# martasumyk/hyperspectral_super-resolution

Measured on AMD Instinct MI355X. Metric: Mpixel*bands/s fused (SRF + deg-3 per-band LSQ fit + apply), higher is better.
Workload: dtype f32

## Files before the change

hyperspectral_super-resolution_amd/csrc/hsr_exec.hip:

```cpp
#include <new>
#include <vector>

#include "hsr_common.h"
#include "hsr_solve.h"
#include "hsr_sync_dev.h"

struct hsr_step_plan {
  hsr_step_desc d;
  int32_t k0[HSR_MAX_BANDS], klen[HSR_MAX_BANDS];
  int32_t slots;
};

enum { kTwoSlot = 0, kFused = 1, kExchange = 2, kGroup = 3 };

struct pipe_slot {
  hsr_step_plan* p = nullptr;
  hipEvent_t ev_k1 = nullptr;
  hipEvent_t ev_fit = nullptr;
  bool pending = false;
  bool fitted = false;
  bool exchanged = false;
  unsigned int seq = 0;
};

struct hsr_pipeline {
  std::vector<pipe_slot> slot;
  int kind = kTwoSlot;
  int nslots = 0;
  int group_T = 0;
  double* group_moments = nullptr;
  double* group_total = nullptr;
  double* group_coeffs = nullptr;
  hipStream_t side = nullptr;
  int64_t n = 0;
  int exchange = 0;
  unsigned int* sync = nullptr;
  unsigned int tickets = 0;
  hsr_exchange x{};
  unsigned int published = 0;
  int deferred = -1;
  int deferred_solve = 0;
  double* host_moments[4] = {};
  struct host_job { hsr_pipeline* pl; double* values; int32_t count; } host_jobs[4] = {};
  volatile int host_error = 0;
};

namespace {

__global__ __launch_bounds__(64) void gate_kernel(const unsigned int* word, unsigned int target, unsigned int* err, unsigned int code) {
  if (threadIdx.x == 0) hsr::wait_word_at_least(word, target, err, code);
}

__global__ __launch_bounds__(64) void publish_add_kernel(unsigned int* word, unsigned int n) {
  if (threadIdx.x == 0) __hip_atomic_fetch_add(word, n, __ATOMIC_RELAXED, __HIP_MEMORY_SCOPE_AGENT);
}

__global__ __launch_bounds__(256) void rehearsal_collective_kernel(int us, unsigned int* sink) {
  __shared__ unsigned int lds[12288];
  lds[threadIdx.x] = threadIdx.x;
  __syncthreads();
  const unsigned long long t0 = hsr::sync_realtime();
  while (hsr::sync_realtime() - t0 < (unsigned long long)us * 100ull) __builtin_amdgcn_s_sleep(8);
  if (lds[(threadIdx.x * 7) & 255] == 0xffffffffu) *sink = 1u;
}

__global__ __launch_bounds__(64) void solve_publish_kernel(const double* __restrict__ moments, int nb, int deg, long long min_count,
                                                           double* coeffs, int do_solve, unsigned int* ready, unsigned int value,
                                                           const unsigned int* gate_word, unsigned int gate_target, unsigned int* err) {
  const int b = threadIdx.x;
  if (do_solve && b < nb) {
    double c[HSR_MAX_DEG + 1];
    hsr::solve_band(moments + (size_t)b * hsr::moment_count(deg), deg, min_count, c);
    for (int j = 0; j <= deg; ++j)
      __hip_atomic_store(coeffs + (size_t)b * (deg + 1) + j, c[j], __ATOMIC_RELAXED, __HIP_MEMORY_SCOPE_AGENT);
  }
  asm volatile("s_waitcnt vmcnt(0)" ::: "memory");
  __syncthreads();
// ... 61 lines not shown

extern "C" int hsr_step_run(hsr_step_plan* p, const void* cube_dev, const float* real_dev, const uint8_t* mask_dev,
                            hsr_stream_t stream) {
  HSR_REQUIRE(p && cube_dev && real_dev, HSR_ERR_INVALID, "hsr_step_run: NULL argument");
  hipStream_t s = (hipStream_t)stream;
  int rc = run_k1(p, cube_dev, real_dev, mask_dev, s);
  if (rc != HSR_OK) return rc;
  rc = hsr_moments_reduce_solve(p->d.partials_dev, p->slots, p->d.nb, p->d.deg, p->d.min_count, p->d.moments_dev, p->d.coeffs_dev, s);
  if (rc != HSR_OK) return rc;
  return run_apply(p, p->d.coeffs_dev, mask_dev, s);
}

extern "C" int hsr_step_run_k1(hsr_step_plan* p, const void* cube_dev, const float* real_dev, const uint8_t* mask_dev,
                               hsr_stream_t stream) {
  HSR_REQUIRE(p && cube_dev && real_dev, HSR_ERR_INVALID, "hsr_step_run_k1: NULL argument");
  return run_k1(p, cube_dev, real_dev, mask_dev, (hipStream_t)stream);
}

extern "C" int hsr_step_run_reduce(hsr_step_plan* p, hsr_stream_t stream) {
  HSR_REQUIRE(p, HSR_ERR_INVALID, "hsr_step_run_reduce: NULL plan");
  return hsr_moments_reduce(p->d.partials_dev, p->slots, p->d.nb, p->d.deg, p->d.moments_dev, stream);
}

extern "C" int hsr_step_run_solve(hsr_step_plan* p, hsr_stream_t stream) {
  HSR_REQUIRE(p, HSR_ERR_INVALID, "hsr_step_run_solve: NULL plan");
  return hsr_poly_solve(p->d.moments_dev, p->d.nb, p->d.deg, p->d.min_count, p->d.coeffs_dev, stream);
}

extern "C" int hsr_step_run_apply(hsr_step_plan* p, const uint8_t* mask_dev, hsr_stream_t stream) {
  HSR_REQUIRE(p, HSR_ERR_INVALID, "hsr_step_run_apply: NULL plan");
  return run_apply(p, p->d.coeffs_dev, mask_dev, (hipStream_t)stream);
}

static int pipeline_new(hsr_step_plan* const* sl, int nslots, int kind, hsr_stream_t side_stream, hsr_pipeline** out, const char* who) {
  HSR_REQUIRE(out, HSR_ERR_INVALID, "%s: NULL argument", who);
  for (int i = 0; i < nslots; ++i) {
    HSR_REQUIRE(sl[i], HSR_ERR_INVALID, "%s: NULL plan", who);
    for (int k = 0; k < i; ++k) {
      HSR_REQUIRE(sl[i] != sl[k], HSR_ERR_INVALID, "%s: distinct plans needed", who);
      const hsr_step_desc &a = sl[i]->d, &b = sl[k]->d;
      HSR_REQUIRE(kind == kTwoSlot || (a.partials_dev != b.partials_dev && a.moments_dev != b.moments_dev && a.coeffs_dev != b.coeffs_dev &&
                                       a.pseudo_dev != b.pseudo_dev && a.matched_dev != b.matched_dev),
                  HSR_ERR_INVALID, "%s: plans %d and %d share a work buffer (partials / moments / coefficients / images must be distinct)", who, k, i);
    }
  }
  HSR_REQUIRE(side_stream != nullptr, HSR_ERR_INVALID, "%s: the side stream must be a real stream, not the default one", who);
  hsr_pipeline* pl = new (std::nothrow) hsr_pipeline();
  HSR_REQUIRE(pl, HSR_ERR_INVALID, "%s: out of host memory", who);
  pl->slot.resize(nslots);
  for (int k = 0; k < nslots; ++k) pl->slot[k].p = sl[k];
  pl->kind = kind;
  pl->nslots = nslots;
  pl->side = (hipStream_t)side_stream;
  bool ok = true;
  if (kind != kTwoSlot)
    ok = hipMalloc(&pl->sync, 8 * sizeof(unsigned int)) == hipSuccess && hipMemset(pl->sync, 0, 8 * sizeof(unsigned int)) == hipSuccess &&
         hipDeviceSynchronize() == hipSuccess;
  if (kind == kTwoSlot || kind == kExchange)
    for (pipe_slot& s : pl->slot)
      ok = ok && hipEventCreateWithFlags(&s.ev_fit, hipEventDisableTiming) == hipSuccess &&
           (kind != kTwoSlot || hipEventCreateWithFlags(&s.ev_k1, hipEventDisableTiming) == hipSuccess);
  if (!ok) {
    (void)hipGetLastError();
    hsr_pipeline_destroy(pl);
    hsr::set_error("%s: could not create the pipeline's device words or events", who);
    return HSR_ERR_HIP;
  }
  *out = pl;
  return HSR_OK;
}

extern "C" int hsr_pipeline_create(hsr_step_plan* slot0, hsr_step_plan* slot1, hsr_stream_t side_stream, int32_t exchange,
                                   hsr_pipeline** out) {
  hsr_step_plan* sl[2] = {slot0, slot1};
  int rc = pipeline_new(sl, 2, kTwoSlot, side_stream, out, "hsr_pipeline_create");
  if (rc == HSR_OK) (*out)->exchange = exchange ? 1 : 0;
  return rc;
}
// ... 44 lines not shown
    for (int k = 0; k < 4; ++k) {
      if (hipHostMalloc(&pl->host_moments[k], bytes, hipHostMallocDefault) != hipSuccess) {
        (void)hipGetLastError();
        hsr_pipeline_destroy(pl);
        hsr::set_error("%s: could not allocate the pinned staging of the host transport", who);
        return HSR_ERR_HIP;
      }
      pl->host_jobs[k] = {pl, pl->host_moments[k], (int32_t)(bytes / sizeof(double))};
    }
  }
  *out = pl;
  return HSR_OK;
}

extern "C" int hsr_pipeline_create_group(hsr_step_plan* const* slots, int32_t nslots, int32_t group_tiles, double* group_moments_dev,
                                         double* group_total_dev, double* group_coeffs_dev, hsr_stream_t side_stream, hsr_pipeline** out) {
  const char* who = "hsr_pipeline_create_group";
  HSR_REQUIRE(slots && out && group_moments_dev && group_total_dev && group_coeffs_dev, HSR_ERR_INVALID, "%s: NULL argument", who);
  HSR_REQUIRE(group_tiles >= 2 && group_tiles <= 64 && nslots == group_tiles + 2, HSR_ERR_INVALID,
              "%s: groups of 2 .. 64 tiles and group_tiles + 2 plans needed (got %d tiles, %d plans)", who, group_tiles, nslots);
  int rc = fused_geometry(slots, nslots, who);
  if (rc != HSR_OK) return rc;
  hsr_pipeline* pl = nullptr;
  rc = pipeline_new(slots, nslots, kGroup, side_stream, &pl, who);
  if (rc != HSR_OK) return rc;
  pl->group_T = group_tiles;
  pl->group_moments = group_moments_dev;
  pl->group_total = group_total_dev;
  pl->group_coeffs = group_coeffs_dev;
  *out = pl;
  return HSR_OK;
}

extern "C" void hsr_pipeline_destroy(hsr_pipeline* pl) {
  if (!pl) return;
  if (pl->kind == kExchange) (void)hipStreamSynchronize(pl->side);
  for (pipe_slot& s : pl->slot) {
    if (s.ev_k1) (void)hipEventDestroy(s.ev_k1);
    if (s.ev_fit) (void)hipEventDestroy(s.ev_fit);
  }
  for (int k = 0; k < 4; ++k)
    if (pl->host_moments[k]) (void)hipHostFree(pl->host_moments[k]);
  if (pl->sync) (void)hipFree(pl->sync);
  delete pl;
}

static inline pipe_slot& slot_of(hsr_pipeline* pl, int64_t tile) { return pl->slot[tile % pl->nslots]; }

static void host_sum_trampoline(void* arg) {
  auto* j = static_cast<hsr_pipeline::host_job*>(arg);
  if (j->pl->x.host_sum(j->pl->x.host_user, j->values, j->count) != 0) j->pl->host_error = 1;
}

static int launch_solve_publish(hsr_pipeline* pl, bool with_gate) {
  const pipe_slot& s = pl->slot[pl->deferred];
  const hsr_step_desc& d = s.p->d;
  hipLaunchKernelGGL(solve_publish_kernel, dim3(1), dim3(64), 0, pl->side, d.moments_dev, d.nb, d.deg, (long long)d.min_count, d.coeffs_dev,
                     pl->deferred_solve, pl->sync + 4 + pl->deferred, s.seq, with_gate ? pl->sync + 1 : nullptr, pl->published, pl->sync + 2);
  HSR_LAUNCH_CHECK("solve_publish_kernel");
  pl->deferred = -1;
  return HSR_OK;
}

static int enqueue_exchange(hsr_pipeline* pl, int k) {
  const hsr_step_desc& d = pl->slot[k].p->d;
  const int64_t nmom = (int64_t)d.nb * hsr::moment_count(d.deg);
  int rc = HSR_OK;
  if (pl->deferred >= 0) {
// ... 180 lines not shown
  rc = run_apply(s.p, s.p->d.coeffs_dev, mask, main);
  s.pending = false;
  return rc;
}

static int submit_two_slot(hsr_pipeline* pl, const void* cube_dev, const float* real_dev, const uint8_t* mask_dev,
                           const uint8_t* prev_mask_dev, hipStream_t main, int32_t* finished_slot, void* k1_begin_event,
                           void* k1_end_event) {
  const int cur = (int)(pl->n % 2);
  pipe_slot &s = pl->slot[cur], &prev = pl->slot[cur ^ 1];
  int rc = HSR_OK;
  if (k1_begin_event) rc = hsr::check_hip(hipEventRecord((hipEvent_t)k1_begin_event, main), "hsr_pipeline: record K1 begin");
  if (rc == HSR_OK) rc = run_k1(s.p, cube_dev, real_dev, mask_dev, main);
  if (rc == HSR_OK && k1_end_event) rc = hsr::check_hip(hipEventRecord((hipEvent_t)k1_end_event, main), "hsr_pipeline: record K1 end");
  if (rc != HSR_OK) return rc;
  if (prev.pending) {
    rc = finish_two_slot(prev, prev_mask_dev, main);
    if (rc != HSR_OK) return rc;
    if (finished_slot) *finished_slot = cur ^ 1;
  }
  rc = hsr::check_hip(hipEventRecord(s.ev_k1, main), "hsr_pipeline: record K1");
  if (rc == HSR_OK) rc = hsr::check_hip(hipStreamWaitEvent(pl->side, s.ev_k1, 0), "hsr_pipeline: side stream wait");
  if (rc == HSR_OK && !pl->exchange) {
    const hsr_step_desc& d = s.p->d;
    rc = hsr_moments_reduce_solve(d.partials_dev, s.p->slots, d.nb, d.deg, d.min_count, d.moments_dev, d.coeffs_dev, pl->side);
    if (rc == HSR_OK) rc = hsr::check_hip(hipEventRecord(s.ev_fit, pl->side), "hsr_pipeline: record fit");
  }
  if (rc != HSR_OK) return rc;
  s.pending = true;
  pl->n += 1;
  return HSR_OK;
}

extern "C" int hsr_pipeline_submit(hsr_pipeline* pl, const void* cube_dev, const float* real_dev, const uint8_t* mask_dev,
                                   const uint8_t* prev_mask_dev, hsr_stream_t main_stream, int32_t* finished_slot,
                                   void* k1_begin_event, void* k1_end_event) {
  HSR_REQUIRE(pl && cube_dev && real_dev, HSR_ERR_INVALID, "hsr_pipeline_submit: NULL argument");
  const int cur = (int)(pl->n % pl->nslots);
  HSR_REQUIRE(!pl->slot[cur].pending, HSR_ERR_INVALID, "hsr_pipeline_submit: slot %d still holds an unfinished tile", cur);
  if (finished_slot) *finished_slot = -1;
  hipStream_t main = (hipStream_t)main_stream;
  if (pl->kind == kTwoSlot) return submit_two_slot(pl, cube_dev, real_dev, mask_dev, prev_mask_dev, main, finished_slot, k1_begin_event, k1_end_event);
  return submit_fused(pl, cube_dev, real_dev, mask_dev, prev_mask_dev, main, finished_slot, k1_begin_event, k1_end_event);
}

extern "C" int hsr_pipeline_fit_done(hsr_pipeline* pl) {
  HSR_REQUIRE(pl && pl->n > 0 && pl->kind == kTwoSlot, HSR_ERR_INVALID, "hsr_pipeline_fit_done: nothing submitted, or not a two-slot pipeline");
  return hsr::check_hip(hipEventRecord(slot_of(pl, pl->n - 1).ev_fit, pl->side), "hsr_pipeline: record fit");
}

extern "C" int hsr_pipeline_flush(hsr_pipeline* pl, const uint8_t* mask_dev, hsr_stream_t main_stream, int32_t* finished_slot) {
  HSR_REQUIRE(pl, HSR_ERR_INVALID, "hsr_pipeline_flush: NULL pipeline");
  if (finished_slot) *finished_slot = -1;
  const int S = pl->nslots;
  for (int64_t i = pl->n >= S - 1 ? pl->n - (S - 1) : 0; i < pl->n; ++i) {
    pipe_slot& s = slot_of(pl, i);
    if (!s.pending) continue;
    const int rc = pl->kind == kTwoSlot ? finish_two_slot(s, mask_dev, (hipStream_t)main_stream)
                                        : finish_fused(pl, i, mask_dev, (hipStream_t)main_stream);
    if (rc == HSR_OK && finished_slot) *finished_slot = (int)(i % S);
    return rc;
  }
  return HSR_OK;
}

extern "C" int64_t hsr_pipeline_count(const hsr_pipeline* pl) { return pl ? pl->n : -1; }

extern "C" int hsr_pipeline_status(hsr_pipeline* pl, hsr_stream_t main_stream, uint32_t* sync_error_out) {
  HSR_REQUIRE(pl && sync_error_out, HSR_ERR_INVALID, "hsr_pipeline_status: NULL argument");
  *sync_error_out = 0;
  int rc = hsr::check_hip(hipStreamSynchronize((hipStream_t)main_stream), "hsr_pipeline_status: caller's stream");
  if (rc == HSR_OK) rc = hsr::check_hip(hipStreamSynchronize(pl->side), "hsr_pipeline_status: side stream");
  if (rc != HSR_OK || !pl->sync) return rc;
  unsigned int code = 0;
  rc = hsr::check_hip(hipMemcpy(&code, pl->sync + 2, sizeof code, hipMemcpyDeviceToHost), "hsr_pipeline_status: read the error word");
  *sync_error_out = code | (pl->host_error ? 16u : 0u);
  return rc;
}
```

hyperspectral_super-resolution_amd/s2_emit/_native.py:

```python
from __future__ import annotations

import ctypes as C
import os
from typing import Optional

_HERE = os.path.dirname(os.path.abspath(__file__))
_DEFAULT_SO = os.path.join(os.path.dirname(_HERE), "lib", "libhsr_mi355x.so")

HSR_OK = 0
HSR_MAX_BANDS = 16
HSR_MAX_DEG = 4
HSR_MAX_APPLY_DEG = 8
HSR_MAX_SPECTRAL = 560
HSR_TILE_PIXELS = 64
HSR_SRF_U16_FAST = 1
HSR_MAX_PARTIALS = 4096
HSR_FIT_GROUPS = 64
HSR_FIT_TICKETS = 65
PLANAR = "planar"
PIXMAJOR = "pixmajor"


class HsrUnavailable(RuntimeError):
    """The HIP extension (or a GPU to run it on) is not available."""
# ... 120 lines not shown
                                _i32, _vp, _vp, _vp, _i32, _vp]),
    "hsr_pair_stats": (C.c_int, [_vp, _vp, _i64, _i32, _vp, _vp, _vp, _vp, _i32, _vp]),
    "hsr_pair_expand_f64": (C.c_int, [_vp, _i64, _vp, _vp, _i64, _vp, _i64, _vp, _i64, _i64, _i32, _i32, _i32, _f64, _vp, _i64,
                                      _i64, _i32, _i32, _vp]),
    "hsr_gram_f64_batched": (C.c_int, [_vp, _i64, _i32, _i32, _i64, _i64, _vp, _i64, _vp, _i64, _i64, _i32, _vp]),
    "hsr_ridge_assemble_batched": (C.c_int, [_vp, _i64, _i64, _i32, _i32, _i32, _f64, _vp, _i32, _i64, _vp, _i64, _i64, _vp, _i32,
                                             _vp]),
    "hsr_chol_solve_f64_batched": (C.c_int, [_vp, _i64, _i32, _i64, _vp, _i64, _i32, _i64, _vp, _vp, _i32, _vp]),
    "hsr_ridge_finish_batched": (C.c_int, [_vp, _i64, _i32, _i32, _i32, _vp, _i64, _i64, _vp, _vp, _i64, _i32, _i32, _vp, _vp,
                                           _i64, _vp, _i64, _vp, _vp, _i64, _vp, _vp, _i32, _vp]),
    "hsr_polyfeat_predict_cube_batched": (C.c_int, [_vp, _i64, _i64, _i64, _vp, _vp, _i64, _i64, _i32, _i32, _vp, _i64, _i64, _vp,
                                                    _i64, _i32, _i32, _i32, _f32, _i32, _vp, _i64, _i64, _i32, _vp]),
    "hsr_pair_report_work_bytes": (C.c_size_t, [_i64, _i32]),
    "hsr_pair_report_f64": (C.c_int, [_vp, _i64, _i64, _i32, _i64, _vp, _i64, _vp, _i64, _i64, _i32, _vp, _i64, _vp, _i64, _i32, _vp,
                                      _vp, _i64, _vp, _vp, _i64, _i32, _vp]),
    "hsr_block_mean": (C.c_int, [_vp, _i32, _i64, _i64, _i32, _i32, _i32, _i32, _f32, _vp, _i64, _i64, _vp]),
    "hsr_bilinear_upsample": (C.c_int, [_vp, _i64, _i64, _i32, _i32, _i32, _i32, _vp, _i64, _i64, _vp]),
    "hsr_bilinear_upsample_mask_hist": (C.c_int, [_vp, _i64, _i64, _i32, _i32, _i32, _i32, _vp, _vp, _vp, _vp]),
    "hsr_probe_read": (C.c_int, [_vp, _i64, _i32, _vp, _vp]),
    "hsr_srf_last_launch": (C.c_int, [_pi32, _pi32, C.POINTER(_i64)]),
    "hsr_srf_kernel_instance": (C.c_int, [_i32, _i32]),
    "hsr_poly_last_launch": (C.c_int, [C.c_char_p, _i32]),
    "hsr_polyfeat_predict_kernel": (C.c_int, [_i32, _i32, _i32, _i32]),
    "hsr_step_plan_create": (C.c_int, [C.POINTER(StepDesc), C.POINTER(_vp)]),
    "hsr_step_plan_destroy": (None, [_vp]),
    "hsr_step_plan_slots": (C.c_int, [_vp]),
    "hsr_step_run": (C.c_int, [_vp, _vp, _vp, _vp, _vp]),
    "hsr_step_run_k1": (C.c_int, [_vp, _vp, _vp, _vp, _vp]),
    "hsr_step_run_reduce": (C.c_int, [_vp, _vp]),
    "hsr_step_run_solve": (C.c_int, [_vp, _vp]),
    "hsr_step_run_apply": (C.c_int, [_vp, _vp, _vp]),
    "hsr_pipeline_create": (C.c_int, [_vp, _vp, _vp, _i32, C.POINTER(_vp)]),
    "hsr_pipeline_create_fused": (C.c_int, [_vp, _vp, _vp, _vp, _i32, C.POINTER(_vp)]),
    "hsr_pipeline_destroy": (None, [_vp]),
    "hsr_pipeline_submit": (C.c_int, [_vp, _vp, _vp, _vp, _vp, _vp, _pi32, _vp, _vp]),
    "hsr_pipeline_fit_done": (C.c_int, [_vp]),
    "hsr_pipeline_flush": (C.c_int, [_vp, _vp, _vp, _pi32]),
    "hsr_pipeline_count": (_i64, [_vp]),
    "hsr_pipeline_create_exchange": (C.c_int, [C.POINTER(_vp), _vp, C.POINTER(Exchange), C.POINTER(_vp)]),
    "hsr_pipeline_status": (C.c_int, [_vp, _vp, C.POINTER(C.c_uint32)]),
    "hsr_pipeline_create_group": (C.c_int, [C.POINTER(_vp), _i32, _i32, _vp, _vp, _vp, _vp, C.POINTER(_vp)]),
    "hsr_srf_fused_launch_supported": (C.c_int, [_i32, _i32, _i32, _pi32, _pi32, _i64, _i32, _popt]),
    "hsr_comm_available": (C.c_int, []),
    "hsr_comm_version": (C.c_int, []),
    "hsr_comm_unique_id": (C.c_int, [_vp]),
    "hsr_comm_init": (C.c_int, [_i32, _i32, _vp, C.POINTER(_vp)]),
    "hsr_comm_destroy": (C.c_int, [_vp]),
    "hsr_comm_rank": (C.c_int, [_vp]),
    "hsr_comm_ranks": (C.c_int, [_vp]),
    "hsr_allreduce_f64": (C.c_int, [_vp, _vp, _i64, _vp]),
    "hsr_reduce_f64": (C.c_int, [_vp, _vp, _i64, _i32, _vp]),
    "hsr_allreduce_u32": (C.c_int, [_vp, _vp, _i64, _vp]),
    "hsr_bcast": (C.c_int, [_vp, _vp, _i64, _i32, _vp]),
}

_lib: Optional[C.CDLL] = None
_lib_path: Optional[str] = None


def library_path() -> str:
    return os.environ.get("HSR_LIBRARY", _DEFAULT_SO)


def load() -> C.CDLL:
    global _lib, _lib_path
    if _lib is not None:
# ... 33 lines not shown
```

hyperspectral_super-resolution_amd/s2_emit/fusion.py:

```python
from __future__ import annotations

from dataclasses import dataclass
from typing import Dict, List, Optional, Tuple

import numpy as np

from . import _engine as eng
from . import _native as nat

COEFF_SYNC_MODES = ("local", "allreduce", "broadcast")
_HOST_GROUPS: Dict[int, object] = {}


def _tkey(t):
    return (t.data_ptr(), tuple(t.shape), tuple(t.stride()), str(t.dtype), str(t.device))


@dataclass
class FusionOutput:
    names: List[str]
    pseudo: object
    moments: object
    coeffs: object
    matched: object
    layout: str = nat.PIXMAJOR

    def band(self, which, image="matched"):
        i = self.names.index(which) if isinstance(which, str) else int(which)
        img = getattr(self, image)
        return img[i] if self.layout == nat.PLANAR else img[:, i]

    def planes(self, image="matched"):
        img = getattr(self, image)
        nb = len(self.names)
        return img if self.layout == nat.PLANAR else img[:, :nb].t().contiguous()


class BatchOutput:

    def __init__(self, names, tb):
        self.names, self._tb = list(names), tb
        self.pseudo, self.matched = tb.pseudo, tb.matched
        self.moments, self.coeffs = tb.moments, tb.coeffs
# ... 4 lines not shown

    def tile(self, i: int) -> FusionOutput:
        tb = self._tb
        return FusionOutput(self.names, tb.tile_rows(i, "pseudo"), tb.moments[i], tb.coeffs[i], tb.tile_rows(i, "matched"),
                            nat.PIXMAJOR)


def exchange_moments(moments, coeffs_solver, group=None, mode: str = "allreduce"):
    import torch.distributed as dist
    if mode not in COEFF_SYNC_MODES:
        raise ValueError(f"mode must be one of {COEFF_SYNC_MODES}, got {mode!r}")
    world = dist.get_world_size(group) if (dist.is_available() and dist.is_initialized()) else 0
    if mode == "local" or world == 0:
        return moments, coeffs_solver(moments)
    if mode == "allreduce":
        dist.all_reduce(moments, op=dist.ReduceOp.SUM, group=group)
        return moments, coeffs_solver(moments)
    root = dist.get_global_rank(group, 0) if group is not None else 0
    dist.reduce(moments, dst=root, op=dist.ReduceOp.SUM, group=group)
    coeffs = coeffs_solver(moments)
    dist.broadcast(coeffs, src=root, group=group)
    return moments, coeffs


class SpectralFusion:

    def __init__(self, emit_w, srf_dict, good_mask=None, deg: int = 3, min_valid: Optional[float] = 0.0,
                 min_count: int = 50, clip: bool = True, apply_mask: bool = False, device=None,
                 group=None, coeff_sync: str = "allreduce", layout: str = nat.PIXMAJOR,
                 force_exchange: bool = False, tile_scale=None, tile_nodata: Optional[int] = eng.TILE_NODATA,
                 reserved_cus: Optional[int] = None, tile_pixels: int = 0, u16_single_buffer: bool = False,
                 u16_fast: bool = False, placement_trials: int = 0, fused_fit: bool = False,
                 placement_pitch_gb: float = eng.PLACEMENT_PITCH_GB, placement_budget_gb: Optional[float] = None,
                 side_stream=None, fuse_apply: bool = False, comm=None, rehearsal_collective=None, group_tiles: int = 1):
        torch = nat.require_gpu()
        self.tile_scale, self.tile_nodata = tile_scale, tile_nodata
        if not 1 <= deg <= nat.HSR_MAX_DEG:
            raise ValueError(f"deg must be in [1, {nat.HSR_MAX_DEG}], got {deg}")
        if coeff_sync not in COEFF_SYNC_MODES:
            raise ValueError(f"coeff_sync must be one of {COEFF_SYNC_MODES}")
        self.device = torch.device(device if device is not None else f"cuda:{torch.cuda.current_device()}")
        self.table = eng.build_srf_table(emit_w, srf_dict, good_mask)
        if self.table.nb == 0:
            raise ValueError("no band of srf_dict has support on the (masked) EMIT wavelength grid")
        if self.table.nb > nat.HSR_MAX_BANDS:
            raise ValueError(f"at most {nat.HSR_MAX_BANDS} supported bands per fusion plan")
        self.deg, self.min_count, self.clip, self.apply_mask = deg, int(min_count), bool(clip), bool(apply_mask)
        self.min_valid = float("-inf") if min_valid is None else float(min_valid)
        self.group, self.coeff_sync = group, coeff_sync
        if layout not in (nat.PIXMAJOR, nat.PLANAR):
            raise ValueError(f"layout must be {nat.PIXMAJOR!r} or {nat.PLANAR!r}")
        self.layout = layout
        self.force_exchange = bool(force_exchange)
        if reserved_cus is None:
            reserved_cus = 8 if self._exchanges() else 0
        self.opts = eng.srf_options(tile_pixels, reserved_cus, u16_single_buffer, u16_fast)
        self.u16_single_buffer = bool(u16_single_buffer)
        self._batches: Dict[tuple, object] = {}
        self.placement_trials = max(0, int(placement_trials))
        self.placement_pitch_gb = float(placement_pitch_gb)
        self.placement_budget_gb = None if placement_budget_gb is None else float(placement_budget_gb)
        self.placement_log: Dict[int, list] = {}
        self._placement_stats: Dict[str, float] = {}
        self.fused_fit = bool(fused_fit)
        self._pipe = None
        self.fused_fallback = None
        self.side_stream = side_stream
        self.side_stream_log = None
        self.fuse_apply = bool(fuse_apply)
        self.group_tiles = int(group_tiles)
        if not 1 <= self.group_tiles <= 64:
            raise ValueError("group_tiles must be in [1, 64]")
        self._comm = comm
        self.rehearsal_collective = rehearsal_collective
        self._host_cb = None
        self._backlog: List[FusionOutput] = []
        self._native: Dict[tuple, object] = {}
        self._native_handles: list = []
        self._pipe_images: Dict[int, list] = {}
        self._pipe_matched: Dict[int, list] = {}
        self.ws = eng.MomentWorkspace(self.device, self.table.nb, deg)
        self.table.device_weights(self.device)
        self._buf: Dict[int, Tuple[object, object]] = {}

    @property
    def names(self) -> List[str]:
        return list(self.table.supported)

    def _buffers(self, npix: int, probe=None):
        torch = nat.require_gpu()
        if npix not in self._buf:
            nb = self.table.nb
            pseudo = eng.alloc_image(torch, nb, npix, self.layout, self.device)
            if probe is not None and self.placement_trials > 1 and npix >= (1 << 16):
                pseudo = self._place(npix, pseudo, probe)
            self._buf[npix] = (pseudo, eng.alloc_image(torch, nb, npix, self.layout, self.device))
        return self._buf[npix]

    @property
    def placement_held_gb(self) -> float:
        return float(self._placement_stats.get("held_gb", 0.0))

    def _trials(self, first, make, probe, cap=None, candidate_bytes: int = 0):
        n = self.placement_trials if cap is None else min(cap, self.placement_trials)
        return eng.placement_search(first, make, probe, n, self.placement_pitch_gb, self.device, self.placement_budget_gb,
                                    candidate_bytes, self._placement_stats)

    def _place(self, npix: int, first, probe, count: int = 1):
        torch = nat.require_gpu()
        nb = self.table.nb
        one = lambda: eng.alloc_image(torch, nb, npix, self.layout, self.device)
        if count == 1:
            keep, times = self._trials(first, one, probe, cap=4, candidate_bytes=first.numel() * 4)
        else:
            keep, times = self._trials(list(first), lambda: [one() for _ in range(count)], lambda c: probe(c[0]), cap=4,
                                       candidate_bytes=count * first[0].numel() * 4)
        self.placement_log[npix] = times
        return keep

    def place_inputs(self, cube, real, mask=None):
        torch = nat.require_gpu()
        npix = cube.numel() // cube.shape[-1]
        if self.placement_trials <= 1 or npix in self._buf:
            return cube, real, {}
        nb = self.table.nb

        def images():
            return [eng.alloc_image(torch, nb, npix, self.layout, self.device) for _ in range(4 if self.fuse_apply else 3)]

        def make():
            return (cube.clone(), real.clone(), images())

        def k1(cand):
            c, r, outs = cand
            rr, rl = self._real_image(r, npix)
            eng.srf_integrate_moments(c, self.table, rr, self.deg, self.ws, mask, self.min_valid, self.min_valid, out=outs[0],
                                      reduce=False, layout=self.layout, real_layout=rl, scale=self.tile_scale,
                                      nodata=self.tile_nodata, opts=self.opts)
        first = (cube, real, images())
        cand_bytes = cube.numel() * cube.element_size() + real.numel() * 4 + 4 * npix * eng.padded_row(nb) * 4
        (cube, real, outs), times = self._trials(first, make, k1, candidate_bytes=cand_bytes)
        self._buf[npix] = (outs[0], eng.alloc_image(torch, nb, npix, self.layout, self.device))
        self._pipe_images[npix] = outs[1:]
        self.placement_log[npix] = times
        return cube, real, {"joint_ms": times}

    def place_mosaic(self, tiles, oversample: float = 12.0, pitch_gb: float = 0.0):
        torch = nat.require_gpu()
        tiles = [(c, r) for c, r in tiles]
        T = len(tiles)
        if self.placement_trials <= 1 or T == 0:
            return tiles, {}
        c0, r0 = tiles[0]
        npix = c0.numel() // c0.shape[-1]
        img = eng.alloc_image(torch, self.table.nb, npix, self.layout, self.device)

        def k1(cand):
            c, r = cand
            rr, rl = self._real_image(r, npix)
            eng.srf_integrate_moments(c, self.table, rr, self.deg, self.ws, None, self.min_valid, self.min_valid, out=img, reduce=False,
                                      layout=self.layout, real_layout=rl, scale=self.tile_scale, nodata=self.tile_nodata, opts=self.opts)
        cand_bytes = c0.numel() * c0.element_size() + r0.numel() * 4
        per = pitch_gb * (1 << 30) + cand_bytes
        free, _ = torch.cuda.mem_get_info(self.device)
        budget = 0.5 * free if self.placement_budget_gb is None else min(self.placement_budget_gb * (1 << 30), free)
        count = int(min(max(T, oversample * T), max(T, budget // per)))
        pitch = pitch_gb
        ranked = eng.placement_rank(lambda: (c0.clone(), r0.clone()), k1, count, pitch, self.device, self.placement_budget_gb, cand_bytes,
                                    self._placement_stats, retime=2 * T)
        ranked += [((c, r), float("inf")) for c, r in tiles[:max(0, T - len(ranked))]]
        order = sorted(range(len(ranked)), key=lambda i: ranked[i][1])[:T]
        kept = []
        for (c, r), i in zip(tiles, order):
# ... 452 lines not shown

    def _pipe_build(self, cube, real, mask, key):
        torch = nat.require_gpu()
        import ctypes as C
        lib = nat.load()
        if self._pipe is not None:
            self._backlog = self.drain()
            old, self._pipe = self._pipe, None
            self._drop_handles(old["handles"])
        npix = cube.numel() // cube.shape[-1]
        real2, real_layout = self._real_image(real, npix)
        if not (real2.is_cuda and real2.dtype == torch.float32):
            raise ValueError("real must be a float32 GPU image with one value per pixel and band")
        eng._as_cube2d(cube)
        nb = self.table.nb

        def probe(img):
            eng.srf_integrate_moments(cube, self.table, real2, self.deg, self.ws, mask, self.min_valid, self.min_valid,
                                      out=img, reduce=False, layout=self.layout, real_layout=real_layout,
                                      scale=self.tile_scale, nodata=self.tile_nodata, opts=self.opts)
        placed = list(self._pipe_images.pop(npix, []))
        if len(placed) < 2:
            placed = [eng.alloc_image(torch, nb, npix, self.layout, self.device) for _ in range(2)]
            if self.placement_trials > 1 and npix >= (1 << 16):
                placed = self._place(npix, placed, probe, count=2)
        exchange = self._exchanges()
        if self.group_tiles > 1 and (exchange or not self.fuse_apply or self.layout != nat.PIXMAJOR):
            raise ValueError("group_tiles > 1 needs fuse_apply=True, the pixel-major layout and no exchange (multi-rank mosaics: fuse_mosaic)")
        if not (self.fuse_apply and self.layout == nat.PIXMAJOR and
                (cube.dtype == torch.float32 or (cube.data_ptr() % 16 == 0 and not self.u16_single_buffer))):
            form = "two"
        else:
            form = "group" if self.group_tiles > 1 else ("exchange" if exchange else "fused")
        nslots = {"two": 2, "fused": 3, "exchange": 4, "group": self.group_tiles + 2}[form]
        while len(placed) < nslots:
            placed.append(eng.alloc_image(torch, nb, npix, self.layout, self.device))
        slots, outs, handles = [], [], []
        placed_m = list(self._pipe_matched.pop(npix, []))
        for k in range(nslots):
            ws = eng.MomentWorkspace(self.device, nb, self.deg)
            matched = placed_m[k] if k < len(placed_m) else eng.alloc_image(torch, nb, npix, self.layout, self.device)
            h, keep = self._native_plan(cube, real2, real_layout, placed[k], matched, ws)
            handles.append(("plan", h))
            slots.append(dict(plan=h, ws=ws, keep=keep, mask=None))
            outs.append(FusionOutput(self.names, placed[k], ws.moments, ws.coeffs, matched, self.layout))
        side = (self.side_stream if self.side_stream is not None else
                torch.cuda.Stream(device=self.device) if form in ("fused", "group") else
                self._pick_side_stream(slots, cube, real2, mask))
        ph = C.c_void_p()
        plans = [sl["plan"] for sl in slots]
        transport = gbuf = None
        if form == "group":
            T, M = self.group_tiles, 3 * self.deg + 2
            gbuf = (torch.zeros((2, T, nb, M), dtype=torch.float64, device=self.device), torch.zeros((2, nb, M), dtype=torch.float64, device=self.device),
                    torch.zeros((2, nb, self.deg + 1), dtype=torch.float64, device=self.device))
            nat.check(lib.hsr_pipeline_create_group((C.c_void_p * nslots)(*plans), nslots, T, gbuf[0].data_ptr(), gbuf[1].data_ptr(),
                                                    gbuf[2].data_ptr(), C.c_void_p(side.cuda_stream), C.byref(ph)), "hsr_pipeline_create_group")
        elif form != "two":
            if form == "exchange":
                x, transport = self._exchange_desc()
                rc = lib.hsr_pipeline_create_exchange((C.c_void_p * 4)(*plans), C.c_void_p(side.cuda_stream), C.byref(x), C.byref(ph))
            else:
                rc = lib.hsr_pipeline_create_fused(*plans, C.c_void_p(side.cuda_stream), 0, C.byref(ph))
            if rc != nat.HSR_OK:
                form, transport = "two", None
                self.fused_fallback = lib.hsr_last_error().decode("utf-8", "replace")
                self._drop_handles(handles[2:])
                slots, outs, handles = slots[:2], outs[:2], handles[:2]
                if self.side_stream is None:
                    side = self._pick_side_stream(slots, cube, real2, mask)
        if form == "two":
            nat.check(lib.hsr_pipeline_create(slots[0]["plan"], slots[1]["plan"], C.c_void_p(side.cuda_stream), 1 if exchange else 0,
                                              C.byref(ph)), "hsr_pipeline_create")
        self._native_handles.append(("pipe", ph))
        handles.append(("pipe", ph))
        self._pipe = dict(key=key, npix=npix, h=ph, slots=slots, outs=outs, side=side, side_handle=C.c_void_p(side.cuda_stream),
                          exchange=exchange, n=0, fin=C.c_int32(-1), fused=form != "two", S=len(slots), inflight=[], handles=handles,
                          c_exchange=form == "exchange", transport=transport, group=gbuf, done=0)
        return self._pipe

    @staticmethod
    def _event_handle(ev, stream):
        if not ev.cuda_event:
            ev.record(stream)
        import ctypes as C
        return C.c_void_p(ev.cuda_event)

    def submit(self, cube, real, mask=None, k1_events=None) -> Optional[FusionOutput]:
        torch = nat.require_gpu()
        import ctypes as C
        lib = nat._lib or nat.load()
        key = (tuple(cube.shape), cube.dtype, tuple(real.shape), tuple(real.stride()), real.dtype,
               cube.dtype == torch.float32 or cube.data_ptr() % 16 == 0)
        st = self._pipe
        if st is None or st["key"] != key:
            st = self._pipe_build(cube, real, mask, key)
        if not (cube.is_contiguous() and cube.device == self.device and real.device == self.device):
            raise ValueError("cube must be a contiguous tensor on the plan's GPU, real on the same GPU")
        if mask is not None and not (mask.dtype == torch.uint8 and mask.numel() == st["npix"] and mask.is_contiguous()
                                     and mask.device == self.device):
            raise ValueError("mask must be a contiguous uint8 tensor with one byte per pixel")
        S = st["S"]
        cur = st["n"] % S
        prev_mask = st["slots"][st["inflight"][0]]["mask"] if len(st["inflight"]) == S - 1 else None
        fin = st["fin"]
        with eng._launch(cube) as stream:
            e0 = e1 = None
            if k1_events is not None:
                ts = torch.cuda.current_stream(self.device)
                e0, e1 = self._event_handle(k1_events[0], ts), self._event_handle(k1_events[1], ts)
            nat.check(lib.hsr_pipeline_submit(st["h"], cube.data_ptr(), real.data_ptr(), None if mask is None else mask.data_ptr(),
                                              None if prev_mask is None else prev_mask.data_ptr(), stream, C.byref(fin), e0, e1),
                      "hsr_pipeline_submit")
            slot = st["slots"][cur]
            slot["mask"] = mask
            slot["ws"].slots = lib.hsr_step_plan_slots(slot["plan"])
            if st["exchange"] and not st["c_exchange"]:
                sh = st["side_handle"]
                with torch.cuda.stream(st["side"]):
                    nat.check(lib.hsr_step_run_reduce(slot["plan"], sh), "hsr_step_run_reduce")

                    def solve(_m, _p=slot["plan"], _ws=slot["ws"]):
                        nat.check(lib.hsr_step_run_solve(_p, sh), "hsr_step_run_solve")
                        return _ws.coeffs
                    exchange_moments(slot["ws"].moments, solve, self.group, self.coeff_sync)
                nat.check(lib.hsr_pipeline_fit_done(st["h"]), "hsr_pipeline_fit_done")
        st["n"] += 1
        st["inflight"].append(cur)
        out = None
        if fin.value >= 0:
            st["inflight"].remove(fin.value)
            st["slots"][fin.value]["mask"] = None
            out = self._finished(st, fin.value)
        if self._backlog:
            if out is not None:
                self._backlog.append(out)
            out = self._backlog.pop(0)
# ... 162 lines not shown
```

include/hsr.h:

```cpp
#ifndef HSR_H_
#define HSR_H_

#include <stddef.h>
#include <stdint.h>

#ifdef __cplusplus
extern "C" {
#endif

#define HSR_ABI_VERSION 5

#define HSR_OK 0
#define HSR_ERR_INVALID 1
#define HSR_ERR_UNSUPPORTED 2
#define HSR_ERR_HIP 3

#define HSR_MAX_BANDS 16
#define HSR_MAX_DEG 4
#define HSR_MAX_APPLY_DEG 8
#define HSR_MAX_SPECTRAL 560
#define HSR_TILE_PIXELS 64
#define HSR_MAX_PARTIALS 4096


// ... 295 lines not shown
  const int32_t* klen;
  int32_t nb, deg;
  float* pseudo_dev;
  int64_t out_bs, out_ps;
  int64_t real_bs, real_ps;
  float min_x, min_y;
  double* partials_dev;
  double* moments_dev;
  double* coeffs_dev;
  int64_t min_count;
  float* matched_dev;
  int64_t matched_bs, matched_ps;
  int32_t apply_mask;
  int32_t clip;
  hsr_srf_options opts;
} hsr_step_desc;
typedef struct hsr_step_plan hsr_step_plan;
typedef struct hsr_pipeline hsr_pipeline;

int hsr_step_plan_create(const hsr_step_desc* desc, hsr_step_plan** plan_out);
void hsr_step_plan_destroy(hsr_step_plan* plan);
int hsr_step_plan_slots(const hsr_step_plan* plan);
int hsr_step_run(hsr_step_plan* plan, const void* cube_dev, const float* real_dev, const uint8_t* mask_dev,
                 hsr_stream_t stream);
int hsr_step_run_k1(hsr_step_plan* plan, const void* cube_dev, const float* real_dev, const uint8_t* mask_dev,
                    hsr_stream_t stream);
int hsr_step_run_reduce(hsr_step_plan* plan, hsr_stream_t stream);
int hsr_step_run_solve(hsr_step_plan* plan, hsr_stream_t stream);
int hsr_step_run_apply(hsr_step_plan* plan, const uint8_t* mask_dev, hsr_stream_t stream);
int hsr_pipeline_create(hsr_step_plan* slot0, hsr_step_plan* slot1, hsr_stream_t side_stream, int32_t exchange,
                        hsr_pipeline** pipeline_out);
int hsr_pipeline_create_fused(hsr_step_plan* slot0, hsr_step_plan* slot1, hsr_step_plan* slot2, hsr_stream_t side_stream,
                              int32_t exchange, hsr_pipeline** pipeline_out);
void hsr_pipeline_destroy(hsr_pipeline* pipeline);
int hsr_pipeline_submit(hsr_pipeline* pipeline, const void* cube_dev, const float* real_dev, const uint8_t* mask_dev,
                        const uint8_t* prev_mask_dev, hsr_stream_t main_stream, int32_t* finished_slot,
                        void* k1_begin_event, void* k1_end_event);
int hsr_pipeline_fit_done(hsr_pipeline* pipeline);
int hsr_pipeline_flush(hsr_pipeline* pipeline, const uint8_t* mask_dev, hsr_stream_t main_stream, int32_t* finished_slot);
int64_t hsr_pipeline_count(const hsr_pipeline* pipeline);

#define HSR_COMM_ID_BYTES 128
typedef struct hsr_comm hsr_comm;
int hsr_comm_available(void);
int hsr_comm_version(void);
int hsr_comm_unique_id(void* id_out);
int hsr_comm_init(int32_t rank, int32_t nranks, const void* unique_id, hsr_comm** comm_out);
int hsr_comm_destroy(hsr_comm* comm);
int hsr_comm_rank(const hsr_comm* comm);
int hsr_comm_ranks(const hsr_comm* comm);
int hsr_allreduce_f64(hsr_comm* comm, double* buf_dev, int64_t count, hsr_stream_t stream);
int hsr_reduce_f64(hsr_comm* comm, double* buf_dev, int64_t count, int32_t root, hsr_stream_t stream);
int hsr_allreduce_u32(hsr_comm* comm, uint32_t* buf_dev, int64_t count, hsr_stream_t stream);
int hsr_bcast(hsr_comm* comm, void* buf_dev, int64_t bytes, int32_t root, hsr_stream_t stream);

#define HSR_SYNC_ALLREDUCE 1
#define HSR_SYNC_BROADCAST 2
typedef int (*hsr_host_sum_fn)(void* user, double* values, int32_t count);
typedef struct hsr_exchange {
  hsr_comm* comm;
  int32_t mode;
  int32_t root;
  hsr_host_sum_fn host_sum;
  void* host_user;
  int32_t rehearsal_us;
  int32_t rehearsal_blocks;
// ... 19 lines not shown
```

Measured before the change: 1.401 million.

## Add two-lane fused pipeline that alternates tiles across independent streams

Adds a 'lanes' pipeline kind that wraps two fused three-slot pipelines, each on its own non-blocking stream, and sends tiles to them alternately. Output is handed back to the caller's stream through events, delayed by one tile. For large tiles it is picked automatically (npix at or above 512K), so the K1, fit and apply work of consecutive tiles can overlap across streams. In exchange it uses six work images and plans instead of three, so memory use roughly doubles, and it adds more event traffic and more complex ordering logic.

After: 1.336 million, median of 2. -4.7%, worse.

```diff
diff --git a/hyperspectral_super-resolution_amd/csrc/hsr_exec.hip b/hyperspectral_super-resolution_amd/csrc/hsr_exec.hip
--- a/hyperspectral_super-resolution_amd/csrc/hsr_exec.hip
+++ b/hyperspectral_super-resolution_amd/csrc/hsr_exec.hip
@@ -11,7 +11,7 @@
   int32_t slots;
 };
 
-enum { kTwoSlot = 0, kFused = 1, kExchange = 2, kGroup = 3 };
+enum { kTwoSlot = 0, kFused = 1, kExchange = 2, kGroup = 3, kLanes = 4 };
 
 struct pipe_slot {
   hsr_step_plan* p = nullptr;
@@ -43,6 +43,14 @@
   double* host_moments[4] = {};
   struct host_job { hsr_pipeline* pl; double* values; int32_t count; } host_jobs[4] = {};
   volatile int host_error = 0;
+  hsr_pipeline* lane[2] = {};
+  hipStream_t lane_stream[2] = {};
+  hipEvent_t ev_in[2] = {};
+  hipEvent_t ev_out[2] = {};
+  hipEvent_t ev_fence = nullptr;
+  int64_t k3 = 0;
+  int held = -1;
+  bool drain_joined = false;
 };
 
 namespace {
@@ -170,8 +178,7 @@
   return run_apply(p, p->d.coeffs_dev, mask_dev, (hipStream_t)stream);
 }
 
-static int pipeline_new(hsr_step_plan* const* sl, int nslots, int kind, hsr_stream_t side_stream, hsr_pipeline** out, const char* who) {
-  HSR_REQUIRE(out, HSR_ERR_INVALID, "%s: NULL argument", who);
+static int distinct_plans(hsr_step_plan* const* sl, int nslots, int kind, const char* who) {
   for (int i = 0; i < nslots; ++i) {
     HSR_REQUIRE(sl[i], HSR_ERR_INVALID, "%s: NULL plan", who);
     for (int k = 0; k < i; ++k) {
@@ -182,6 +189,13 @@
                   HSR_ERR_INVALID, "%s: plans %d and %d share a work buffer (partials / moments / coefficients / images must be distinct)", who, k, i);
     }
   }
+  return HSR_OK;
+}
+
+static int pipeline_new(hsr_step_plan* const* sl, int nslots, int kind, hsr_stream_t side_stream, hsr_pipeline** out, const char* who) {
+  HSR_REQUIRE(out, HSR_ERR_INVALID, "%s: NULL argument", who);
+  const int distinct = distinct_plans(sl, nslots, kind, who);
+  if (distinct != HSR_OK) return distinct;
   HSR_REQUIRE(side_stream != nullptr, HSR_ERR_INVALID, "%s: the side stream must be a real stream, not the default one", who);
   hsr_pipeline* pl = new (std::nothrow) hsr_pipeline();
   HSR_REQUIRE(pl, HSR_ERR_INVALID, "%s: out of host memory", who);
@@ -292,8 +306,53 @@
   return HSR_OK;
 }
 
+extern "C" int hsr_pipeline_create_lanes(hsr_step_plan* const* slots6, hsr_pipeline** out) {
+  const char* who = "hsr_pipeline_create_lanes";
+  HSR_REQUIRE(slots6 && out, HSR_ERR_INVALID, "%s: NULL argument", who);
+  int rc = fused_geometry(slots6, 6, who);
+  if (rc == HSR_OK) rc = distinct_plans(slots6, 6, kLanes, who);
+  if (rc != HSR_OK) return rc;
+  hsr_pipeline* pl = new (std::nothrow) hsr_pipeline();
+  HSR_REQUIRE(pl, HSR_ERR_INVALID, "%s: out of host memory", who);
+  pl->kind = kLanes;
+  pl->nslots = 6;
+  bool ok = hipEventCreateWithFlags(&pl->ev_fence, hipEventDisableTiming) == hipSuccess;
+  for (int l = 0; l < 2 && ok; ++l)
+    ok = hipStreamCreateWithFlags(&pl->lane_stream[l], hipStreamNonBlocking) == hipSuccess &&
+         hipEventCreateWithFlags(&pl->ev_in[l], hipEventDisableTiming) == hipSuccess &&
+         hipEventCreateWithFlags(&pl->ev_out[l], hipEventDisableTiming) == hipSuccess;
+  if (!ok) {
+    (void)hipGetLastError();
+    hsr_pipeline_destroy(pl);
+    hsr::set_error("%s: could not create the lanes' streams or events", who);
+    return HSR_ERR_HIP;
+  }
+  for (int l = 0; l < 2; ++l) {
+    hsr_step_plan* ps[3] = {slots6[l], slots6[l + 2], slots6[l + 4]};
+    rc = pipeline_new(ps, 3, kFused, pl->lane_stream[l], &pl->lane[l], who);
+    if (rc != HSR_OK) {
+      hsr_pipeline_destroy(pl);
+      return rc;
+    }
+  }
+  *out = pl;
+  return HSR_OK;
+}
+
 extern "C" void hsr_pipeline_destroy(hsr_pipeline* pl) {
   if (!pl) return;
+  if (pl->kind == kLanes) {
+    for (int l = 0; l < 2; ++l) {
+      if (pl->lane_stream[l]) (void)hipStreamSynchronize(pl->lane_stream[l]);
+      hsr_pipeline_destroy(pl->lane[l]);
+      if (pl->ev_in[l]) (void)hipEventDestroy(pl->ev_in[l]);
+      if (pl->ev_out[l]) (void)hipEventDestroy(pl->ev_out[l]);
+      if (pl->lane_stream[l]) (void)hipStreamDestroy(pl->lane_stream[l]);
+    }
+    if (pl->ev_fence) (void)hipEventDestroy(pl->ev_fence);
+    delete pl;
+    return;
+  }
   if (pl->kind == kExchange) (void)hipStreamSynchronize(pl->side);
   for (pipe_slot& s : pl->slot) {
     if (s.ev_k1) (void)hipEventDestroy(s.ev_k1);
@@ -540,10 +599,71 @@
   return HSR_OK;
 }
 
+static int lanes_hand_out(hsr_pipeline* pl, hipStream_t main, int32_t* finished_slot) {
+  const int rc = hsr::check_hip(hipStreamWaitEvent(main, pl->ev_out[pl->held & 1], 0), "hsr_pipeline: wait for the lane");
+  if (rc != HSR_OK) return rc;
+  if (finished_slot) *finished_slot = pl->held;
+  pl->held = -1;
+  return HSR_OK;
+}
+
+static int lanes_k3_enqueued(hsr_pipeline* pl, int l, int lane_slot) {
+  const int rc = hsr::check_hip(hipEventRecord(pl->ev_out[l], pl->lane_stream[l]), "hsr_pipeline: record the lane");
+  if (rc != HSR_OK) return rc;
+  pl->held = l + 2 * lane_slot;
+  pl->k3 += 1;
+  return HSR_OK;
+}
+
+static int submit_lanes(hsr_pipeline* pl, const void* cube_dev, const float* real_dev, const uint8_t* mask_dev,
+                        const uint8_t* prev_mask_dev, hipStream_t main, int32_t* finished_slot, void* k1_begin_event,
+                        void* k1_end_event) {
+  const int l = (int)(pl->n & 1);
+  hipStream_t ls = pl->lane_stream[l];
+  int rc = hsr::check_hip(hipEventRecord(pl->ev_in[l], main), "hsr_pipeline: record the caller's stream");
+  if (rc == HSR_OK) rc = hsr::check_hip(hipStreamWaitEvent(ls, pl->ev_in[l], 0), "hsr_pipeline: lane waits for the inputs");
+  if (rc == HSR_OK && (k1_begin_event || k1_end_event)) {
+    rc = hsr::check_hip(hipEventRecord(pl->ev_fence, pl->lane_stream[l ^ 1]), "hsr_pipeline: record the other lane");
+    if (rc == HSR_OK) rc = hsr::check_hip(hipStreamWaitEvent(ls, pl->ev_fence, 0), "hsr_pipeline: lane waits for the other lane");
+  }
+  if (rc != HSR_OK) return rc;
+  int32_t fin = -1;
+  rc = hsr_pipeline_submit(pl->lane[l], cube_dev, real_dev, mask_dev, prev_mask_dev, ls, &fin, k1_begin_event, k1_end_event);
+  if (rc != HSR_OK) return rc;
+  pl->n += 1;
+  pl->drain_joined = false;
+  if (pl->held >= 0) rc = lanes_hand_out(pl, main, finished_slot);
+  if (rc == HSR_OK && fin >= 0) rc = lanes_k3_enqueued(pl, l, fin);
+  return rc;
+}
+
+static int flush_lanes(hsr_pipeline* pl, const uint8_t* mask_dev, hipStream_t main, int32_t* finished_slot) {
+  if (pl->held >= 0) return lanes_hand_out(pl, main, finished_slot);
+  if (pl->k3 >= pl->n) return HSR_OK;
+  int rc = HSR_OK;
+  for (int l = 0; l < 2 && !pl->drain_joined && rc == HSR_OK; ++l) {
+    rc = hsr::check_hip(hipEventRecord(pl->ev_in[l], main), "hsr_pipeline: record the caller's stream");
+    if (rc == HSR_OK) rc = hsr::check_hip(hipStreamWaitEvent(pl->lane_stream[l], pl->ev_in[l], 0), "hsr_pipeline: lane waits for the caller");
+  }
+  if (rc != HSR_OK) return rc;
+  pl->drain_joined = true;
+  const int l = (int)(pl->k3 & 1);
+  int32_t fin = -1;
+  rc = hsr_pipeline_flush(pl->lane[l], mask_dev, pl->lane_stream[l], &fin);
+  if (rc != HSR_OK) return rc;
+  HSR_REQUIRE(fin >= 0, HSR_ERR_INVALID, "hsr_pipeline_flush: lane %d holds no unfinished tile, %lld expected", l, (long long)pl->k3);
+  rc = lanes_k3_enqueued(pl, l, fin);
+  return rc == HSR_OK ? lanes_hand_out(pl, main, finished_slot) : rc;
+}
+
 extern "C" int hsr_pipeline_submit(hsr_pipeline* pl, const void* cube_dev, const float* real_dev, const uint8_t* mask_dev,
                                    const uint8_t* prev_mask_dev, hsr_stream_t main_stream, int32_t* finished_slot,
                                    void* k1_begin_event, void* k1_end_event) {
   HSR_REQUIRE(pl && cube_dev && real_dev, HSR_ERR_INVALID, "hsr_pipeline_submit: NULL argument");
+  if (pl->kind == kLanes) {
+    if (finished_slot) *finished_slot = -1;
+    return submit_lanes(pl, cube_dev, real_dev, mask_dev, prev_mask_dev, (hipStream_t)main_stream, finished_slot, k1_begin_event, k1_end_event);
+  }
   const int cur = (int)(pl->n % pl->nslots);
   HSR_REQUIRE(!pl->slot[cur].pending, HSR_ERR_INVALID, "hsr_pipeline_submit: slot %d still holds an unfinished tile", cur);
   if (finished_slot) *finished_slot = -1;
@@ -560,6 +680,7 @@
 extern "C" int hsr_pipeline_flush(hsr_pipeline* pl, const uint8_t* mask_dev, hsr_stream_t main_stream, int32_t* finished_slot) {
   HSR_REQUIRE(pl, HSR_ERR_INVALID, "hsr_pipeline_flush: NULL pipeline");
   if (finished_slot) *finished_slot = -1;
+  if (pl->kind == kLanes) return flush_lanes(pl, mask_dev, (hipStream_t)main_stream, finished_slot);
   const int S = pl->nslots;
   for (int64_t i = pl->n >= S - 1 ? pl->n - (S - 1) : 0; i < pl->n; ++i) {
     pipe_slot& s = slot_of(pl, i);
@@ -578,7 +699,9 @@
   HSR_REQUIRE(pl && sync_error_out, HSR_ERR_INVALID, "hsr_pipeline_status: NULL argument");
   *sync_error_out = 0;
   int rc = hsr::check_hip(hipStreamSynchronize((hipStream_t)main_stream), "hsr_pipeline_status: caller's stream");
-  if (rc == HSR_OK) rc = hsr::check_hip(hipStreamSynchronize(pl->side), "hsr_pipeline_status: side stream");
+  for (int l = 0; l < 2 && rc == HSR_OK && pl->kind == kLanes; ++l)
+    rc = hsr::check_hip(hipStreamSynchronize(pl->lane_stream[l]), "hsr_pipeline_status: lane");
+  if (rc == HSR_OK && pl->kind != kLanes) rc = hsr::check_hip(hipStreamSynchronize(pl->side), "hsr_pipeline_status: side stream");
   if (rc != HSR_OK || !pl->sync) return rc;
   unsigned int code = 0;
   rc = hsr::check_hip(hipMemcpy(&code, pl->sync + 2, sizeof code, hipMemcpyDeviceToHost), "hsr_pipeline_status: read the error word");
diff --git a/hyperspectral_super-resolution_amd/s2_emit/_native.py b/hyperspectral_super-resolution_amd/s2_emit/_native.py
--- a/hyperspectral_super-resolution_amd/s2_emit/_native.py
+++ b/hyperspectral_super-resolution_amd/s2_emit/_native.py
@@ -176,6 +176,7 @@
     "hsr_step_run_apply": (C.c_int, [_vp, _vp, _vp]),
     "hsr_pipeline_create": (C.c_int, [_vp, _vp, _vp, _i32, C.POINTER(_vp)]),
     "hsr_pipeline_create_fused": (C.c_int, [_vp, _vp, _vp, _vp, _i32, C.POINTER(_vp)]),
+    "hsr_pipeline_create_lanes": (C.c_int, [C.POINTER(_vp), C.POINTER(_vp)]),
     "hsr_pipeline_destroy": (None, [_vp]),
     "hsr_pipeline_submit": (C.c_int, [_vp, _vp, _vp, _vp, _vp, _vp, _pi32, _vp, _vp]),
     "hsr_pipeline_fit_done": (C.c_int, [_vp]),
diff --git a/hyperspectral_super-resolution_amd/s2_emit/fusion.py b/hyperspectral_super-resolution_amd/s2_emit/fusion.py
--- a/hyperspectral_super-resolution_amd/s2_emit/fusion.py
+++ b/hyperspectral_super-resolution_amd/s2_emit/fusion.py
@@ -9,6 +9,7 @@
 from . import _native as nat
 
 COEFF_SYNC_MODES = ("local", "allreduce", "broadcast")
+TWO_LANE_MIN_PIXELS = 512 * 1024
 _HOST_GROUPS: Dict[int, object] = {}
 
 
@@ -79,7 +80,8 @@
                  reserved_cus: Optional[int] = None, tile_pixels: int = 0, u16_single_buffer: bool = False,
                  u16_fast: bool = False, placement_trials: int = 0, fused_fit: bool = False,
                  placement_pitch_gb: float = eng.PLACEMENT_PITCH_GB, placement_budget_gb: Optional[float] = None,
-                 side_stream=None, fuse_apply: bool = False, comm=None, rehearsal_collective=None, group_tiles: int = 1):
+                 side_stream=None, fuse_apply: bool = False, comm=None, rehearsal_collective=None, group_tiles: int = 1,
+                 lanes: Optional[int] = None):
         torch = nat.require_gpu()
         self.tile_scale, self.tile_nodata = tile_scale, tile_nodata
         if not 1 <= deg <= nat.HSR_MAX_DEG:
@@ -118,6 +120,9 @@
         self.group_tiles = int(group_tiles)
         if not 1 <= self.group_tiles <= 64:
             raise ValueError("group_tiles must be in [1, 64]")
+        if lanes not in (None, 1, 2):
+            raise ValueError("lanes must be None (automatic), 1 or 2")
+        self.lanes = lanes
         self._comm = comm
         self.rehearsal_collective = rehearsal_collective
         self._host_cb = None
@@ -172,8 +177,10 @@
             return cube, real, {}
         nb = self.table.nb
 
+        nimg = 3 if not self.fuse_apply else 7 if (self.group_tiles == 1 and not self._exchanges() and self._lanes_for(npix) == 2) else 4
+
         def images():
-            return [eng.alloc_image(torch, nb, npix, self.layout, self.device) for _ in range(4 if self.fuse_apply else 3)]
+            return [eng.alloc_image(torch, nb, npix, self.layout, self.device) for _ in range(nimg)]
 
         def make():
             return (cube.clone(), real.clone(), images())
@@ -185,7 +192,7 @@
                                       reduce=False, layout=self.layout, real_layout=rl, scale=self.tile_scale,
                                       nodata=self.tile_nodata, opts=self.opts)
         first = (cube, real, images())
-        cand_bytes = cube.numel() * cube.element_size() + real.numel() * 4 + 4 * npix * eng.padded_row(nb) * 4
+        cand_bytes = cube.numel() * cube.element_size() + real.numel() * 4 + nimg * npix * eng.padded_row(nb) * 4
         (cube, real, outs), times = self._trials(first, make, k1, candidate_bytes=cand_bytes)
         self._buf[npix] = (outs[0], eng.alloc_image(torch, nb, npix, self.layout, self.device))
         self._pipe_images[npix] = outs[1:]
@@ -704,7 +711,9 @@
             form = "two"
         else:
             form = "group" if self.group_tiles > 1 else ("exchange" if exchange else "fused")
-        nslots = {"two": 2, "fused": 3, "exchange": 4, "group": self.group_tiles + 2}[form]
+            if form == "fused" and self._lanes_for(npix) == 2:
+                form = "lanes"
+        nslots = {"two": 2, "fused": 3, "lanes": 6, "exchange": 4, "group": self.group_tiles + 2}[form]
         while len(placed) < nslots:
             placed.append(eng.alloc_image(torch, nb, npix, self.layout, self.device))
         slots, outs, handles = [], [], []
@@ -717,7 +726,7 @@
             slots.append(dict(plan=h, ws=ws, keep=keep, mask=None))
             outs.append(FusionOutput(self.names, placed[k], ws.moments, ws.coeffs, matched, self.layout))
         side = (self.side_stream if self.side_stream is not None else
-                torch.cuda.Stream(device=self.device) if form in ("fused", "group") else
+                torch.cuda.Stream(device=self.device) if form in ("fused", "lanes", "group") else
                 self._pick_side_stream(slots, cube, real2, mask))
         ph = C.c_void_p()
         plans = [sl["plan"] for sl in slots]
@@ -732,6 +741,8 @@
             if form == "exchange":
                 x, transport = self._exchange_desc()
                 rc = lib.hsr_pipeline_create_exchange((C.c_void_p * 4)(*plans), C.c_void_p(side.cuda_stream), C.byref(x), C.byref(ph))
+            elif form == "lanes":
+                rc = lib.hsr_pipeline_create_lanes((C.c_void_p * 6)(*plans), C.byref(ph))
             else:
                 rc = lib.hsr_pipeline_create_fused(*plans, C.c_void_p(side.cuda_stream), 0, C.byref(ph))
             if rc != nat.HSR_OK:
@@ -748,8 +759,14 @@
         handles.append(("pipe", ph))
         self._pipe = dict(key=key, npix=npix, h=ph, slots=slots, outs=outs, side=side, side_handle=C.c_void_p(side.cuda_stream),
                           exchange=exchange, n=0, fin=C.c_int32(-1), fused=form != "two", S=len(slots), inflight=[], handles=handles,
-                          c_exchange=form == "exchange", transport=transport, group=gbuf, done=0)
+                          c_exchange=form == "exchange", transport=transport, group=gbuf, done=0, lanes=2 if form == "lanes" else 1,
+                          k3_depth=4 if form == "lanes" else len(slots) - 1)
         return self._pipe
+
+    def _lanes_for(self, npix: int) -> int:
+        if self.lanes is not None:
+            return self.lanes
+        return 2 if npix >= TWO_LANE_MIN_PIXELS else 1
 
     @staticmethod
     def _event_handle(ev, stream):
@@ -774,7 +791,7 @@
             raise ValueError("mask must be a contiguous uint8 tensor with one byte per pixel")
         S = st["S"]
         cur = st["n"] % S
-        prev_mask = st["slots"][st["inflight"][0]]["mask"] if len(st["inflight"]) == S - 1 else None
+        prev_mask = st["slots"][(st["n"] - st["k3_depth"]) % S]["mask"] if st["n"] >= st["k3_depth"] else None
         fin = st["fin"]
         with eng._launch(cube) as stream:
             e0 = e1 = None
diff --git a/include/hsr.h b/include/hsr.h
--- a/include/hsr.h
+++ b/include/hsr.h
@@ -351,6 +351,7 @@
                         hsr_pipeline** pipeline_out);
 int hsr_pipeline_create_fused(hsr_step_plan* slot0, hsr_step_plan* slot1, hsr_step_plan* slot2, hsr_stream_t side_stream,
                               int32_t exchange, hsr_pipeline** pipeline_out);
+int hsr_pipeline_create_lanes(hsr_step_plan* const* slots6, hsr_pipeline** pipeline_out);
 void hsr_pipeline_destroy(hsr_pipeline* pipeline);
 int hsr_pipeline_submit(hsr_pipeline* pipeline, const void* cube_dev, const float* real_dev, const uint8_t* mask_dev,
                         const uint8_t* prev_mask_dev, hsr_stream_t main_stream, int32_t* finished_slot,
```
